# miloknowles/adaptive-stereo-icra-2021

Measured on AMD Instinct MI355X. Metric: stereo pairs/sec (fwd+adapt-step), KITTI 1242x375 D=192, higher is better.
Workload: dtype f32; 1 GPU; KITTI-2015 1242x375, maxdisp 192, k=4 (Dc=12, 24x78 cost volume), forward + one online-adapt step (train-mode BN, monodepth loss, clip 1.0, Adam lr 5e-5); pairs_per_gpu=4, global_batch=4, parallelism=dp1 (per-replica BatchNorm statistics, one flat RCCL gradient all-reduce), kernels=all hand-written HIP (no MIOpen/rocBLAS on the path)

## Files before the change

adaptive-stereo-icra-2021_amd/csrc/conv32_mfma.hip:

```cpp
#include "as_common.h"
#include "conv_epilogue.h"
#include <cstdlib>
#include "conv3d_lds.h"

struct ConvArgs {
  const float* x;
  const float* wp;
  EpilogueArgs ep;
  PclDev gin, gout;
  ConvMap map;
  int M;
  int ntaps;
  int tap_off[AS_MAX_TAPS];
};

__device__ inline void load16(f32x4 (&r)[4], const float* p) {
  const f32x4* q = reinterpret_cast<const f32x4*>(p);
  r[0] = q[0]; r[1] = q[1]; r[2] = q[2]; r[3] = q[3];
}

__device__ inline void loadw(f32x4 (&r)[4], const float* p) {
  r[0] = *reinterpret_cast<const f32x4*>(p);
  r[1] = *reinterpret_cast<const f32x4*>(p + 256);
  r[2] = *reinterpret_cast<const f32x4*>(p + 512);
  r[3] = *reinterpret_cast<const f32x4*>(p + 768);
}

__device__ inline void mfma16(f32x16& acc, const f32x4 (&a)[4], const f32x4 (&b)[4]) {
#pragma unroll
  for (int q = 0; q < 4; ++q) {
    acc = __builtin_amdgcn_mfma_f32_32x32x2f32(a[q].x, b[q].x, acc, 0, 0, 0);
    acc = __builtin_amdgcn_mfma_f32_32x32x2f32(a[q].y, b[q].y, acc, 0, 0, 0);
    acc = __builtin_amdgcn_mfma_f32_32x32x2f32(a[q].z, b[q].z, acc, 0, 0, 0);
    acc = __builtin_amdgcn_mfma_f32_32x32x2f32(a[q].w, b[q].w, acc, 0, 0, 0);
  }
}

#ifndef AS_CONV32_PREFETCH
#define AS_CONV32_PREFETCH 1
#endif
template <int NT>
__device__ __forceinline__ void conv32_fwd_body(const ConvArgs& p, const int block, float (*red)[32], float* bmean) {
  const int lane = threadIdx.x & 63, wave = threadIdx.x >> 6;
  const int h = lane >> 5, li = lane & 31;
  const int tile = block * 4 + wave;
  const int v = tile * 32 + li;
  const bool valid = v < p.M;
  int in_vox, out_vox;
  conv_decode(valid ? v : p.M - 1, p.gin, p.gout, p.map, in_vox, out_vox);

  const float* xa = p.x + (long)in_vox * 32 + h * 16;
  const float* wb = p.wp + lane * 4;

  const float bias_v = p.ep.bias[li];
  __builtin_amdgcn_sched_barrier(0);

  constexpr int PF = AS_CONV32_PREFETCH, RING = PF + 1;
  f32x4 a[RING][4], b[RING][4];
#pragma unroll
  for (int tp = 0; tp < PF && tp < NT; ++tp) {
    load16(a[tp % RING], xa + (long)p.tap_off[tp] * 32);
    loadw(b[tp % RING], wb + tp * 1024);
    __builtin_amdgcn_sched_barrier(0);
  }
  f32x16 acc;
#pragma unroll
  for (int r = 0; r < 16; ++r) acc[r] = bias_v;
#pragma unroll
  for (int tp = 0; tp < NT; ++tp) {
    if (tp + PF < NT) {
      load16(a[(tp + PF) % RING], xa + (long)p.tap_off[tp + PF] * 32);
      loadw(b[(tp + PF) % RING], wb + (tp + PF) * 1024);
    }
    __builtin_amdgcn_sched_barrier(0);
    mfma16(acc, a[tp % RING], b[tp % RING]);
    __builtin_amdgcn_sched_barrier(0);
  }
  TileStats ts;
  conv_epilogue(acc, p.ep, out_vox, valid, min(128, p.M - block * 128), red, bmean, &ts);
  stats_write(p.ep, block, ts);
}

template <int NT>
__global__ __launch_bounds__(256) void conv32_fwd_kernel(ConvArgs p) {
  __shared__ float red[4][32];
  __shared__ float bmean[32];
  conv32_fwd_body<NT>(p, (int)blockIdx.x, red, bmean);
}

struct DgradS2Args { ConvArgs ph[4]; int nblk[4]; };

__global__ __launch_bounds__(256) void conv32_dgrad_s2_kernel(DgradS2Args p) {
  __shared__ float red[4][32];
  __shared__ float bmean[32];
  int b = (int)blockIdx.x;
  if (b < p.nblk[0]) { conv32_fwd_body<9>(p.ph[0], b, red, bmean); return; }
  b -= p.nblk[0];
  if (b < p.nblk[1]) { conv32_fwd_body<6>(p.ph[1], b, red, bmean); return; }
  b -= p.nblk[1];
  if (b < p.nblk[2]) { conv32_fwd_body<6>(p.ph[2], b, red, bmean); return; }
  b -= p.nblk[2];
  conv32_fwd_body<4>(p.ph[3], b, red, bmean);
}

#ifndef CONV32_SPLITK_MAX_M
#define CONV32_SPLITK_MAX_M 32768
#endif
bool conv32_splitk_applies(int ntaps, int64_t M) {
  return (ntaps == 9 && M <= CONV32_SPLITK_MAX_M) || (ntaps == 25 && M <= CONV32_SPLITK_MAX_M / 2);
}

template <int NT>
__global__ __launch_bounds__(256) void conv32_fwd_splitk_kernel(ConvArgs p) {
  __shared__ float red[4][32];
  __shared__ float bmean[32];
  __shared__ float part[3][16][64];
  const int lane = threadIdx.x & 63, wave = __builtin_amdgcn_readfirstlane(threadIdx.x >> 6);
  const int h = lane >> 5, li = lane & 31;
  const int v = blockIdx.x * 32 + li;
  const bool in_range = v < p.M;
  int in_vox, out_vox;
  conv_decode(in_range ? v : p.M - 1, p.gin, p.gout, p.map, in_vox, out_vox);
  const float* xa = p.x + (long)in_vox * 32 + h * 16;
  const float* wb = p.wp + lane * 4;
  const float bias_v = wave == 0 ? p.ep.bias[li] : 0.f;
  constexpr int PER = (NT + 3) / 4;
  f32x4 a[2][4], b[2][4];
  if (wave < NT) {
    load16(a[0], xa + (long)p.tap_off[wave] * 32);
    loadw(b[0], wb + wave * 1024);
  }
  f32x16 acc;
#pragma unroll
  for (int r = 0; r < 16; ++r) acc[r] = bias_v;
#pragma unroll
  for (int k = 0; k < PER; ++k) {
    const int tp = wave + 4 * k;
    if (k + 1 < PER && tp + 4 < NT) {
      load16(a[(k + 1) & 1], xa + (long)p.tap_off[tp + 4] * 32);
      loadw(b[(k + 1) & 1], wb + (tp + 4) * 1024);
    }
    __builtin_amdgcn_sched_barrier(0);
    if (tp < NT) mfma16(acc, a[k & 1], b[k & 1]);
    __builtin_amdgcn_sched_barrier(0);
  }
  if (wave > 0) {
#pragma unroll
    for (int r = 0; r < 16; ++r) part[wave - 1][r][lane] = acc[r];
  }
  __syncthreads();
  if (wave == 0) {
#pragma unroll
    for (int r = 0; r < 16; ++r) acc[r] = ((acc[r] + part[0][r][lane]) + part[1][r][lane]) + part[2][r][lane];
  }
  TileStats ts;
  conv_epilogue(acc, p.ep, out_vox, in_range && wave == 0, min(32, p.M - (int)blockIdx.x * 32), red, bmean, &ts);
  stats_write(p.ep, blockIdx.x, ts);
}

__global__ void pack_weights_kernel(const float* __restrict__ w, float* __restrict__ packed, int T, int flip) {
  const int idx = blockIdx.x * blockDim.x + threadIdx.x;
  if (idx >= T * 1024) return;
  const int e = idx & 3, j = (idx >> 2) & 31, h = (idx >> 7) & 1, q = (idx >> 8) & 3, t = idx >> 10;
  const int k = 16 * h + 4 * q + e;
  float v;
  if (!flip) v = w[((long)j * 32 + k) * T + t];
  else       v = w[((long)k * 32 + j) * T + (T - 1 - t)];
  packed[idx] = v;
}

#define WG_SEG_STEPS 32
template <int TG>
struct WgradAcc { f32x16 a[TG]; };

struct WgradArgs {
  const float* x;
  const float* gz;
  float* partial;
  float* partial_db;
  PclDev gin, gout;
  int rows;
  int nseg;
  int seg_steps;
  int rows_per_chunk;
  int nchunks;
  int ntaps;
  int stride;
  int tap_off[AS_MAX_TAPS];
};

template <int TG>
__global__ __launch_bounds__(256) void conv32_wgrad_kernel(WgradArgs p) {
  extern __shared__ __attribute__((aligned(16))) float lds[];
  const int lane = threadIdx.x & 63, wave = threadIdx.x >> 6;
  const int h = lane >> 5, li = lane & 31;
  int group, chunk;
  {
    const int ngroups = p.ntaps / TG;
    const int L = blockIdx.x, xcd = L & 7, q = L >> 3;
    const int per_xcd = (p.nchunks + 7) >> 3;
    group = q % ngroups;
    chunk = xcd * per_xcd + q / ngroups;
    if (chunk >= p.nchunks || q / ngroups >= per_xcd) return;
  }
  const int W = p.gout.W, H = p.gout.H, D = p.gout.D;
  const int r0 = chunk * p.rows_per_chunk;
  const int r1 = min(p.rows, r0 + p.rows_per_chunk);

  f32x16 acc[TG];
#pragma unroll
  for (int g = 0; g < TG; ++g)
#pragma unroll
    for (int r = 0; r < 16; ++r) acc[g][r] = 0.f;
  float bsum = 0.f;

  int toff[TG];
#pragma unroll
  for (int g = 0; g < TG; ++g) toff[g] = p.tap_off[group * TG + g] * 32;

  constexpr int WG_U = 8;
  const int nsteps = (W + 1) >> 1;
  const int xs = 32 * p.stride;
  for (int unit = r0 + wave; unit < r1; unit += 4) {
    const int row = unit / p.nseg, seg = unit - row * p.nseg;
    int t = row;
    const int y = t % H; t /= H;
    const int d = t % D;
    const int b = t / D;
    const float* xr = p.x + p.gin.vox(b, d, y * p.stride, 0) * 32 + li;
    const float* gr = p.gz + p.gout.vox(b, d, y, 0) * 32 + li;
    const int s_end = min(nsteps, (seg + 1) * p.seg_steps);
    for (int s0 = seg * p.seg_steps; s0 < s_end; s0 += WG_U) {
      float bv[WG_U], av[WG_U][TG];
#pragma unroll
      for (int u = 0; u < WG_U; ++u) {
        const int xc = 2 * (s0 + u) + h;
        const bool ok = xc < W;
        const int xcl = ok ? xc : W - 1;
#ifdef WG_EXP_NOLOAD
        const float g0 = (float)(xcl + lane);
        bv[u] = ok ? g0 : 0.f;
#pragma unroll
        for (int g = 0; g < TG; ++g) av[u][g] = (float)(xcl * xs + toff[g]);
#else
        const float g0 = gr[xcl * 32];
        bv[u] = ok ? g0 : 0.f;
#pragma unroll
        for (int g = 0; g < TG; ++g) av[u][g] = xr[xcl * xs + toff[g]];
#endif
      }
      __builtin_amdgcn_sched_barrier(0);
#pragma unroll
      for (int u = 0; u < WG_U; ++u) {
        bsum += bv[u];
#pragma unroll
        for (int g = 0; g < TG; ++g)
#ifdef WG_EXP_NOMFMA
          acc[g][0] += av[u][g] * bv[u];
#else
          acc[g] = __builtin_amdgcn_mfma_f32_32x32x2f32(av[u][g], bv[u], acc[g], 0, 0, 0);
#endif
      }
    }
  }

  float* slab = lds;
  float* dbs = lds + 3 * TG * 16 * 64;
  bsum += __shfl_xor(bsum, 32, 64);
  if (h == 0) dbs[wave * 32 + li] = bsum;
  if (wave > 0) {
#pragma unroll
    for (int g = 0; g < TG; ++g)
#pragma unroll
      for (int r = 0; r < 16; ++r) slab[((wave - 1) * TG * 16 + g * 16 + r) * 64 + lane] = acc[g][r];
  }
  __syncthreads();
  if (wave == 0) {
#pragma unroll
    for (int g = 0; g < TG; ++g) {
      const int tap = group * TG + g;
      float* out = p.partial + ((long)chunk * p.ntaps + tap) * 1024;
#pragma unroll
      for (int r = 0; r < 16; ++r) {
        float v = acc[g][r];
        v += slab[(0 * TG * 16 + g * 16 + r) * 64 + lane];
        v += slab[(1 * TG * 16 + g * 16 + r) * 64 + lane];
        v += slab[(2 * TG * 16 + g * 16 + r) * 64 + lane];
        const int ci = (r & 3) + 8 * (r >> 2) + 4 * h;
        out[ci * 32 + li] = v;
      }
    }
    if (group == 0 && h == 0)
      p.partial_db[chunk * 32 + li] = dbs[li] + dbs[32 + li] + dbs[64 + li] + dbs[96 + li];
  }
}

__global__ __launch_bounds__(1024) void wgrad_reduce_kernel(const float* __restrict__ partial,
                                                             const float* __restrict__ partial_db, int nchunks, int T,
                                                             float* __restrict__ dW, float* __restrict__ db, int accumulate) {
  __shared__ float red[16][64];
  const int o = threadIdx.x & 63, sl = threadIdx.x >> 6;
  const int total = T * 1024;
  const int idx = blockIdx.x * 64 + o;
  const bool is_w = idx < total, is_b = !is_w && db != nullptr && idx < total + 32;
  float s = 0.f;
  if (is_w) {
    const float* src = partial + idx;
#pragma unroll 8
    for (int c = sl; c < nchunks; c += 16) s += src[(long)c * total];
  } else if (is_b) {
    const float* src = partial_db + (idx - total);
#pragma unroll 8
    for (int c = sl; c < nchunks; c += 16) s += src[c * 32];
  }
  red[sl][o] = s;
  __syncthreads();
  if (sl == 0 && (is_w || is_b)) {
    float t = 0.f;
#pragma unroll
    for (int k = 0; k < 16; ++k) t += red[k][o];
    if (is_w) {
      const int oc = idx & 31, i = (idx >> 5) & 31, tp = idx >> 10;
      float* dst = dW + ((long)oc * 32 + i) * T + tp;
      *dst = accumulate ? *dst + t : t;
    } else {
      db[idx - total] = accumulate ? db[idx - total] + t : t;
    }
  }
}

struct ReduceJob { const float* partial; const float* partial_db; int nchunks, accumulate; };
#define RB_MAX_DEST 32
#define RB_MAX_JOBS 2
struct ReduceDest { float* dW; float* db; int T, njobs; ReduceJob job[RB_MAX_JOBS]; };
struct ReduceBatch { int ndest; ReduceDest dest[RB_MAX_DEST]; };

__global__ __launch_bounds__(1024) void wgrad_reduce_batch_kernel(ReduceBatch rb) {
  __shared__ f32x4 red[16][64];
  const ReduceDest& d = rb.dest[blockIdx.y];
  const int o = threadIdx.x & 63, sl = threadIdx.x >> 6;
  const int total = d.T * 1024;
  const int idx = (blockIdx.x * 64 + o) * 4;
  if (blockIdx.x * 256 >= total + 32) return;
  const bool is_w = idx < total, is_b = !is_w && d.db != nullptr && idx < total + 32;
  f32x4 v = {0.f, 0.f, 0.f, 0.f};
  bool have = false;
  for (int j = 0; j < d.njobs; ++j) {
    const ReduceJob& jb = d.job[j];
    f32x4 s = {0.f, 0.f, 0.f, 0.f};
    if (is_w) {
      const float* src = jb.partial + idx;
#pragma unroll 8
      for (int c = sl; c < jb.nchunks; c += 16) s += *reinterpret_cast<const f32x4*>(src + (long)c * total);
    } else if (is_b) {
      const float* src = jb.partial_db + (idx - total);
#pragma unroll 8
      for (int c = sl; c < jb.nchunks; c += 16) s += *reinterpret_cast<const f32x4*>(src + c * 32);
    }
    __syncthreads();
    red[sl][o] = s;
    __syncthreads();
    if (sl == 0 && (is_w || is_b)) {
      f32x4 t = {0.f, 0.f, 0.f, 0.f};
#pragma unroll
      for (int k = 0; k < 16; ++k) t += red[k][o];
      if (jb.accumulate) {
        if (!have) {
#pragma unroll
          for (int e = 0; e < 4; ++e) {
            const int id = idx + e;
            v[e] = is_w ? d.dW[((long)(id & 31) * 32 + ((id >> 5) & 31)) * d.T + (id >> 10)] : d.db[id - total];
          }
          have = true;
        }
        v = v + t;
      } else { v = t; have = true; }
    }
  }
  if (sl == 0 && (is_w || is_b)) {
#pragma unroll
    for (int e = 0; e < 4; ++e) {
      const int id = idx + e;
      if (is_w) d.dW[((long)(id & 31) * 32 + ((id >> 5) & 31)) * d.T + (id >> 10)] = v[e];
      else d.db[id - total] = v[e];
    }
  }
}

#include <mutex>
#include <vector>
struct PendingReduce { const float* partial; const float* partial_db; int nchunks, T; float* dW; float* db; int accumulate; };
static std::mutex g_defer_mutex;
static bool g_defer_on = false;
static std::vector<PendingReduce> g_defer_jobs;

void as_wgrad_reduce_enqueue(hipStream_t st, const float* partial, const float* partial_db, int nchunks, int T, float* dW,
                             float* db, int accumulate) {
  {
    std::lock_guard<std::mutex> lock(g_defer_mutex);
    if (g_defer_on && accumulate) { g_defer_jobs.push_back({partial, partial_db, nchunks, T, dW, db, accumulate}); return; }
  }
  hipLaunchKernelGGL(wgrad_reduce_kernel, dim3(as_div_up(T * 1024 + 32, 64)), dim3(1024), 0, st, partial, partial_db, nchunks, T,
                     dW, db, accumulate);
}

extern "C" int as_wgrad_defer(int on) {
  std::lock_guard<std::mutex> lock(g_defer_mutex);
  const int prev = g_defer_on ? 1 : 0;
  g_defer_on = on != 0;
  return prev;
}

extern "C" int as_wgrad_defer_pending(void) {
  std::lock_guard<std::mutex> lock(g_defer_mutex);
  return (int)g_defer_jobs.size();
}

static void launch_reduce_batch(const ReduceBatch& rb, hipStream_t st) {
  int tmax = 0;
  for (int i = 0; i < rb.ndest; ++i) tmax = rb.dest[i].T > tmax ? rb.dest[i].T : tmax;
  hipLaunchKernelGGL(wgrad_reduce_batch_kernel, dim3(as_div_up(tmax * 1024 + 32, 256), rb.ndest), dim3(1024), 0, st, rb);
}

extern "C" int as_wgrad_defer_flush(void* stream) {
  std::vector<PendingReduce> jobs;
  {
    std::lock_guard<std::mutex> lock(g_defer_mutex);
    jobs.swap(g_defer_jobs);
  }
  hipStream_t st = (hipStream_t)stream;
  ReduceBatch rb;
  rb.ndest = 0;
  for (const PendingReduce& pj : jobs) {
    int di = -1;
    for (int i = 0; i < rb.ndest; ++i) if (rb.dest[i].dW == pj.dW) di = i;
    if (di >= 0 && (rb.dest[di].njobs == RB_MAX_JOBS || rb.dest[di].T != pj.T || rb.dest[di].db != pj.db)) {
      launch_reduce_batch(rb, st);
      rb.ndest = 0; di = -1;
    }
    if (di < 0) {
      if (rb.ndest == RB_MAX_DEST) { launch_reduce_batch(rb, st); rb.ndest = 0; }
      di = rb.ndest++;
      rb.dest[di].dW = pj.dW; rb.dest[di].db = pj.db; rb.dest[di].T = pj.T; rb.dest[di].njobs = 0;
    }
    ReduceJob& jb = rb.dest[di].job[rb.dest[di].njobs++];
    jb.partial = pj.partial; jb.partial_db = pj.partial_db; jb.nchunks = pj.nchunks; jb.accumulate = pj.accumulate;
  }
// ... 103 lines not shown
    for (int px = 0; px < 2; ++px, ++ph) {
      const int Hl = (ggx->H - py + 1) / 2, Wl = (ggx->W - px + 1) / 2;
      ConvArgs& a = args.ph[ph];
      int n = 0;
      for (int j = py; j < 5; j += 2)
        for (int l = px; l < 5; l += 2) {
          a.tap_off[n] = ((py + 2 - j) / 2) * Wp + (px + 2 - l) / 2;
          ++n;
        }
      a.x = f.x; a.wp = wp; a.ep = epilogue_args(f);
      a.gin = as_make_dev(ggz); a.gout = as_make_dev(ggx);
      a.map.Hl = Hl > 0 ? Hl : 1; a.map.Wl = Wl > 0 ? Wl : 1; a.map.in_stride = 1; a.map.out_stride = 2; a.map.out_oy = py; a.map.out_ox = px;
      a.M = (Hl > 0 && Wl > 0) ? ggx->B * Hl * Wl : 0; a.ntaps = n;
      args.nblk[ph] = as_div_up(a.M, 128);
      total += args.nblk[ph];
      wp += n * 1024;
    }
  if (total > 0) hipLaunchKernelGGL(conv32_dgrad_s2_kernel, dim3(total), dim3(256), 0, (hipStream_t)stream, args);
  return AS_OK;
}

extern "C" int as_conv32_pack_weights(const float* w, float* packed, const as_conv_shape* s,
                                      int transpose_flip, void* stream) {
  AS_CHECK_ARG(w && packed && s, "as_conv32_pack_weights: null pointer");
  const int T = s->kd * s->kh * s->kw;
  AS_CHECK_ARG(T >= 1 && T <= AS_MAX_TAPS, "as_conv32_pack_weights: %d taps unsupported", T);
  hipLaunchKernelGGL(pack_weights_kernel, dim3(as_div_up(T * 1024, 256)), dim3(256), 0, (hipStream_t)stream,
                     w, packed, T, transpose_flip);
  AS_CHECK_LAUNCH("as_conv32_pack_weights");
  return AS_OK;
}

__device__ inline int s2_phase_major_tap(int t) {
  int n = 0;
  for (int py = 0; py < 2; ++py)
    for (int px = 0; px < 2; ++px)
      for (int j = py; j < 5; j += 2)
        for (int l = px; l < 5; l += 2) { if (n == t) return j * 5 + l; ++n; }
  return 0;
}

__device__ inline float wino_g_row(int r, float x0, float x1, float x2) {
  return r == 0 ? x0 : (r == 3 ? x2 : (r == 1 ? 0.5f * ((x0 + x2) + x1) : 0.5f * ((x0 + x2) - x1)));
}
__device__ inline void wino_pack_one(const float* __restrict__ w, float* __restrict__ packed, int idx, bool transposed) {
  if (idx >= 16 * 1024) return;
  const int e = idx & 3, j = (idx >> 2) & 31, h = (idx >> 7) & 1, q = (idx >> 8) & 3, kk = idx >> 10;
  const int k = 16 * h + 4 * q + e, r = kk >> 2, c = kk & 3;
  const float* g = transposed ? w + ((long)k * 32 + j) * 9 : w + ((long)j * 32 + k) * 9;
  float col[3];
#pragma unroll
  for (int a = 0; a < 3; ++a) {
    const float* ga = g + 3 * (transposed ? 2 - a : a);
    col[a] = transposed ? wino_g_row(c, ga[2], ga[1], ga[0]) : wino_g_row(c, ga[0], ga[1], ga[2]);
  }
  packed[idx] = wino_g_row(r, col[0], col[1], col[2]);
}
__global__ void wino_pack_kernel(const float* __restrict__ w, float* __restrict__ packed, int transposed) {
  wino_pack_one(w, packed, blockIdx.x * blockDim.x + threadIdx.x, transposed != 0);
}

__global__ void pack_weights_batch_kernel(const as_pack_job* __restrict__ jobs) {
  const as_pack_job job = jobs[blockIdx.y];
  const int T = job.taps, kind = job.transpose_flip;
  const int idx = blockIdx.x * blockDim.x + threadIdx.x;
  if (kind >= AS_PACK_CONV4 && kind < AS_PACK_CONV4 + 8) {
    const int Cin = kind - AS_PACK_CONV4;
    if (idx >= T * 128) return;
    const int co = idx & 31, h = (idx >> 5) & 1, j = (idx >> 6) & 1, t = idx >> 7;
    const int c = 2 * j + h;
    job.packed[idx] = c < Cin ? job.w[((long)co * Cin + c) * T + t] : 0.f;
    return;
  }
  if (kind == AS_PACK_MIRROR_TAP || kind == AS_PACK_MIRROR_CH) {
    if (idx >= 288) return;
    const int c = idx / 9, t = idx - 9 * c;
    const float v = job.w[((long)c * 4) * 9 + (8 - t)];
    job.packed[kind == AS_PACK_MIRROR_TAP ? t * 32 + c : c * 9 + t] = v;
    return;
  }
  if (kind == AS_PACK_WINO || kind == AS_PACK_WINO_T) { wino_pack_one(job.w, job.packed, idx, kind == AS_PACK_WINO_T); return; }
  if (idx >= T * 1024) return;
  const int e = idx & 3, j = (idx >> 2) & 31, h = (idx >> 7) & 1, q = (idx >> 8) & 3, t = idx >> 10;
  const int k = 16 * h + 4 * q + e;
  if (kind == AS_PACK_S2_DGRAD) job.packed[idx] = job.w[((long)k * 32 + j) * T + s2_phase_major_tap(t)];
  else job.packed[idx] = kind ? job.w[((long)k * 32 + j) * T + (T - 1 - t)] : job.w[((long)j * 32 + k) * T + t];
}

extern "C" int as_conv32_pack_weights_batch(const as_pack_job* jobs, int njobs, int max_taps, void* stream) {
  AS_CHECK_ARG(jobs && njobs >= 1 && njobs <= 65535, "as_conv32_pack_weights_batch: bad job table");
  AS_CHECK_ARG(max_taps >= 1 && max_taps <= AS_MAX_TAPS, "as_conv32_pack_weights_batch: %d taps unsupported", max_taps);
  hipLaunchKernelGGL(pack_weights_batch_kernel, dim3(as_div_up(max_taps * 1024, 256), njobs), dim3(256), 0,
                     (hipStream_t)stream, jobs);
  AS_CHECK_LAUNCH("as_conv32_pack_weights_batch");
  return AS_OK;
}

extern "C" int as_conv32_wino_pack_weights(const float* w, float* packed, int transposed, void* stream) {
  AS_CHECK_ARG(w && packed, "as_conv32_wino_pack_weights: null pointer");
  hipLaunchKernelGGL(wino_pack_kernel, dim3(64), dim3(256), 0, (hipStream_t)stream, w, packed, transposed);
  AS_CHECK_LAUNCH("as_conv32_wino_pack_weights");
  return AS_OK;
}

extern "C" int as_conv3d_wgrad_lds_assignment(int ntiles, int nchunks, int block, int* chunk, int* kd, int* extra_tile) {
  AS_CHECK_ARG(chunk && kd && extra_tile && ntiles >= 1 && nchunks >= 1 && nchunks <= ntiles && block >= 0,
               "as_conv3d_wgrad_lds_assignment: bad arguments");
  return conv3d_wgrad_assign(block, ntiles, nchunks, chunk, kd, extra_tile) ? 1 : 0;
}

Wgrad32Plan conv32_wgrad_plan(const as_pcl* gout, const as_conv_shape* s) {
  Wgrad32Plan p;
  p.T = s->kd * s->kh * s->kw;
  p.tap_group = (p.T % 3 == 0) ? 3 : (p.T % 5 == 0 ? 5 : 1);
  const int groups = p.T / p.tap_group;
  const int nsteps = (gout->W + 1) >> 1;
  const long waves = (long)gout->B * gout->D * gout->H * groups;
  int nseg = 1;
  if (waves < 1024) {
    nseg = (int)((2048 + waves - 1) / waves);
    const int most = (nsteps + WG_SEG_STEPS - 1) / WG_SEG_STEPS;
    if (nseg > most) nseg = most;
    if (nseg < 1) nseg = 1;
  }
  int steps = (nsteps + nseg - 1) / nseg;
  p.seg_steps = (steps + 7) / 8 * 8;
  p.nseg = (nsteps + p.seg_steps - 1) / p.seg_steps;
  const int rows = gout->B * gout->D * gout->H * p.nseg;
  int want_chunks = (4096 + groups * 4 - 1) / (groups * 4);
  if (want_chunks > 512) want_chunks = 512;
  p.rows_per_chunk = (rows + want_chunks - 1) / want_chunks;
  if (p.rows_per_chunk < 4) p.rows_per_chunk = 4;
  p.nchunks = (rows + p.rows_per_chunk - 1) / p.rows_per_chunk;
  return p;
}

template <int TG>
static void launch_wgrad(const WgradArgs& a, int groups, int nchunks, hipStream_t st) {
  const size_t lds = (size_t)(3 * TG * 16 * 64 + 4 * 32) * sizeof(float);
  const int per_xcd = (nchunks + 7) / 8;
  hipLaunchKernelGGL(conv32_wgrad_kernel<TG>, dim3(8 * per_xcd * groups), dim3(256), lds, st, a);
}

int conv32_wgrad_generic_launch(const ConvWgradArgs& w, const as_pcl* gin, const as_pcl* gout, const as_conv_shape* s,
                                const Wgrad32Plan& p, const char* who, void* stream) {
  WgradArgs a;
  a.x = w.x; a.gz = w.gz; a.partial = w.partial; a.partial_db = w.partial_db;
  a.gin = as_make_dev(gin); a.gout = as_make_dev(gout);
  a.nseg = p.nseg; a.seg_steps = p.seg_steps;
  a.rows = gout->B * gout->D * gout->H * a.nseg; a.rows_per_chunk = p.rows_per_chunk; a.nchunks = p.nchunks; a.ntaps = p.T;
  a.stride = s->stride;
  if (int e = fill_taps(gin, s, a.tap_off, who)) return e;
  hipStream_t st = (hipStream_t)stream;
  if (p.tap_group == 3) launch_wgrad<3>(a, p.T / 3, p.nchunks, st);
  else if (p.tap_group == 5) launch_wgrad<5>(a, p.T / 5, p.nchunks, st);
  else launch_wgrad<1>(a, p.T, p.nchunks, st);
  return AS_OK;
}
```

adaptive-stereo-icra-2021_amd/csrc/conv32_s2.hip:

```cpp
#include "as_common.h"
#include "conv_entry.h"

struct S2Args {
  const float* x;
  const float* wp;
  const float* bias;
  float* out;
  PclDev gin, gout;
  int nseg, ntiles;
};

__device__ inline void s2_loadw(f32x4 (&r)[4], const float* p) {
  r[0] = *reinterpret_cast<const f32x4*>(p);
  r[1] = *reinterpret_cast<const f32x4*>(p + 256);
  r[2] = *reinterpret_cast<const f32x4*>(p + 512);
  r[3] = *reinterpret_cast<const f32x4*>(p + 768);
}
__device__ inline void s2_mfma16(f32x16& acc, const f32x4 (&a)[4], const f32x4 (&b)[4]) {
#pragma unroll
  for (int q = 0; q < 4; ++q) {
    acc = __builtin_amdgcn_mfma_f32_32x32x2f32(a[q].x, b[q].x, acc, 0, 0, 0);
    acc = __builtin_amdgcn_mfma_f32_32x32x2f32(a[q].y, b[q].y, acc, 0, 0, 0);
    acc = __builtin_amdgcn_mfma_f32_32x32x2f32(a[q].z, b[q].z, acc, 0, 0, 0);
    acc = __builtin_amdgcn_mfma_f32_32x32x2f32(a[q].w, b[q].w, acc, 0, 0, 0);
  }
}

#define S2F_HALF (36 * 128)
#define S2F_BUF (2 * S2F_HALF)
#define S2F_WAVE (2 * S2F_BUF)

__global__ __launch_bounds__(256, 2) void conv32_s2_fwd_kernel(S2Args p) {
  extern __shared__ __attribute__((aligned(16))) char smem_s2[];
  const int lane = threadIdx.x & 63, wave = threadIdx.x >> 6;
  const int h = lane >> 5, li = lane & 31;
  const int tile = blockIdx.x * 4 + wave;
  if (tile >= p.ntiles) return;
  const int seg = tile % p.nseg, row = tile / p.nseg;
  const int y = row % p.gout.H, b = row / p.gout.H;
  const int x0 = seg * 32;
  char* buf = smem_s2 + wave * S2F_WAVE;

  const int sv = lane >> 3, sq = lane & 7;
  const int s_half = (sv & 1) * S2F_HALF;
  const float* src0 = p.x + ((((long)b * p.gin.Hp + (2 * y - 2 + p.gin.ph)) * p.gin.Wp + (2 * x0 - 2 + p.gin.pw)) * 32) + sq * 4;
  const int vlim = p.gin.Wp - 1 - (2 * x0 - 2 + p.gin.pw);
  int voff[9];
#pragma unroll
  for (int i = 0; i < 9; ++i) voff[i] = min(8 * i + sv, vlim) * 32;
  auto fetch = [&](f32x4 (&r)[9], int ky) {
    const float* src = src0 + (long)ky * p.gin.Wp * 32;
#pragma unroll
    for (int i = 0; i < 9; ++i) r[i] = *reinterpret_cast<const f32x4*>(src + voff[i]);
  };
  auto stage = [&](const f32x4 (&r)[9], char* dst) {
#pragma unroll
    for (int i = 0; i < 9; ++i) {
      const int e = 4 * i + (sv >> 1);
      *reinterpret_cast<f32x4*>(dst + s_half + e * 128 + ((sq ^ ((e >> 1) & 7)) << 4)) = r[i];
    }
  };
  const float* wb = p.wp + lane * 4;
  const float bias_v = p.bias ? p.bias[li] : 0.f;
  f32x16 acc;
#pragma unroll
  for (int r = 0; r < 16; ++r) acc[r] = bias_v;

  f32x4 ra[9], rb[9];
  f32x4 bw[2][4];
  fetch(ra, 0);
  s2_loadw(bw[0], wb);
#pragma unroll
  for (int ky = 0; ky < 5; ++ky) {
    char* cur = buf + (ky & 1) * S2F_BUF;
    if (ky & 1) stage(rb, cur); else stage(ra, cur);
    if (ky + 1 < 5) { if (ky & 1) fetch(ra, ky + 1); else fetch(rb, ky + 1); }
#pragma unroll
    for (int kx = 0; kx < 5; ++kx) {
      const int tp = ky * 5 + kx;
      if (tp + 1 < 25) s2_loadw(bw[(tp + 1) & 1], wb + (tp + 1) * 1024);
      f32x4 a[4];
      const int e = li + (kx >> 1);
      const char* ap = cur + (kx & 1) * S2F_HALF + e * 128;
      const int sw = (e >> 1) & 7;
#pragma unroll
      for (int q = 0; q < 4; ++q) a[q] = *reinterpret_cast<const f32x4*>(ap + (((4 * h + q) ^ sw) << 4));
      __builtin_amdgcn_sched_barrier(0);
      s2_mfma16(acc, a, bw[tp & 1]);
      __builtin_amdgcn_sched_barrier(0);
    }
  }
  float* outp = p.out + ((((long)b * p.gout.Hp + (y + p.gout.ph)) * p.gout.Wp + (x0 + p.gout.pw)) * 32) + li;
#pragma unroll
  for (int r = 0; r < 16; ++r) {
    const int xo = (r & 3) + 8 * (r >> 2) + 4 * h;
    if (x0 + xo < p.gout.W) outp[xo * 32] = acc[r];
  }
}

bool conv32_s2_fwd_applicable(const as_pcl* gin, const as_pcl* gout, const as_conv_shape* s) {
  if (s->kd != 1 || s->kh != 5 || s->kw != 5 || s->stride != 2 || s->dil != 1 || s->pad_h != 2 || s->pad_w != 2) return false;
  if (gin->D != 1 || gout->D != 1 || gin->pd != 0 || gin->B != gout->B) return false;
  if (gout->H != (gin->H - 1) / 2 + 1 || gout->W != (gin->W - 1) / 2 + 1) return false;
  if (gin->ph < 2 || gin->pw < 2) return false;
  return (long)gout->B * gout->H * ((gout->W + 31) / 32) >= 1024;
}

int conv32_s2_fwd_launch(const ConvFwdArgs& f, const as_pcl* gin, const as_pcl* gout, const as_conv_shape*, const char* who,
                         void* stream) {
  static AsPerDevice attr_set;
  S2Args a;
  a.x = f.x; a.wp = f.w; a.bias = f.bias; a.out = f.z; a.gin = as_make_dev(gin); a.gout = as_make_dev(gout);
  a.nseg = (gout->W + 31) / 32; a.ntiles = gout->B * gout->H * a.nseg;
  void* kargs[] = {&a};
  return as_launch_lds(reinterpret_cast<const void*>(conv32_s2_fwd_kernel), attr_set, 4 * S2F_WAVE, 4 * S2F_WAVE,
                       dim3(as_div_up(a.ntiles, 4)), dim3(256), kargs, who, (hipStream_t)stream);
}

#define S2D_ROW (40 * 128)
#define S2D_WAVE (3 * S2D_ROW)

__global__ __launch_bounds__(256, 2) void conv32_s2_dgrad_kernel(S2Args p) {
  extern __shared__ __attribute__((aligned(16))) char smem_s2[];
  const int lane = threadIdx.x & 63, wave = threadIdx.x >> 6;
  const int h = lane >> 5, li = lane & 31;
  const int tile = blockIdx.x * 4 + wave;
  if (tile >= p.ntiles) return;
  const int seg = tile % p.nseg, row = tile / p.nseg;
  const int yc = row % p.gin.H, b = row / p.gin.H;
  const int x0 = seg * 32;
  char* buf = smem_s2 + wave * S2D_WAVE;

  const int sv = lane >> 3, sq = lane & 7;
  const float* src0 = p.x + ((((long)b * p.gin.Hp + (yc - 1 + p.gin.ph)) * p.gin.Wp + (x0 - 1 + p.gin.pw)) * 32) + sq * 4;
  const int vlim = p.gin.Wp - 1 - (x0 - 1 + p.gin.pw);
  int voff[5];
#pragma unroll
  for (int i = 0; i < 5; ++i) voff[i] = min(8 * i + sv, vlim) * 32;
  f32x4 r[3][5];
#pragma unroll
  for (int dy = 0; dy < 3; ++dy)
#pragma unroll
    for (int i = 0; i < 5; ++i) r[dy][i] = *reinterpret_cast<const f32x4*>(src0 + (long)dy * p.gin.Wp * 32 + voff[i]);
  const float* wb = p.wp + lane * 4;
  f32x4 bw[2][4];
  s2_loadw(bw[0], wb);
#pragma unroll
  for (int dy = 0; dy < 3; ++dy)
#pragma unroll
    for (int i = 0; i < 5; ++i) {
      const int e = 8 * i + sv;
      *reinterpret_cast<f32x4*>(buf + dy * S2D_ROW + e * 128 + ((sq ^ ((e >> 1) & 7)) << 4)) = r[dy][i];
    }

  int tp = 0;
#pragma unroll
  for (int ph = 0; ph < 4; ++ph) {
    const int py = ph >> 1, px = ph & 1;
    f32x16 acc;
#pragma unroll
    for (int rr = 0; rr < 16; ++rr) acc[rr] = 0.f;
#pragma unroll
    for (int j = py; j < 5; j += 2)
#pragma unroll
      for (int l = px; l < 5; l += 2, ++tp) {
        if (tp + 1 < 25) s2_loadw(bw[(tp + 1) & 1], wb + (tp + 1) * 1024);
        const int dy = (py + 2 - j) / 2 + 1, dx = (px + 2 - l) / 2;
        const int e = li + 1 + dx;
        const char* ap = buf + dy * S2D_ROW + e * 128;
        const int sw = (e >> 1) & 7;
        f32x4 a[4];
#pragma unroll
        for (int q = 0; q < 4; ++q) a[q] = *reinterpret_cast<const f32x4*>(ap + (((4 * h + q) ^ sw) << 4));
        __builtin_amdgcn_sched_barrier(0);
        s2_mfma16(acc, a, bw[tp & 1]);
        __builtin_amdgcn_sched_barrier(0);
      }
    const int yo = 2 * yc + py;
    if (yo < p.gout.H) {
      float* outp = p.out + ((((long)b * p.gout.Hp + (yo + p.gout.ph)) * p.gout.Wp + (2 * x0 + px + p.gout.pw)) * 32) + li;
#pragma unroll
      for (int rr = 0; rr < 16; ++rr) {
        const int xo = (rr & 3) + 8 * (rr >> 2) + 4 * h;
        if (2 * (x0 + xo) + px < p.gout.W) outp[xo * 64] = acc[rr];
      }
    }
  }
}

bool conv32_s2_dgrad_applicable(const as_pcl* ggz, const as_pcl* ggx) {
  if (ggz->D != 1 || ggx->D != 1 || ggz->B != ggx->B || ggz->pd != 0) return false;
  if (ggz->H != (ggx->H - 1) / 2 + 1 || ggz->W != (ggx->W - 1) / 2 + 1) return false;
  if (ggz->ph < 1 || ggz->pw < 1) return false;
  return (long)ggz->B * ggz->H * ((ggz->W + 31) / 32) >= 1024;
}

int conv32_s2_dgrad_launch(const float* gz, const as_pcl* ggz, const float* packed, float* gx, const as_pcl* ggx, const char* who,
                           void* stream) {
  static AsPerDevice attr_set;
  S2Args a;
  a.x = gz; a.wp = packed; a.bias = nullptr; a.out = gx; a.gin = as_make_dev(ggz); a.gout = as_make_dev(ggx);
  a.nseg = (ggz->W + 31) / 32; a.ntiles = ggz->B * ggz->H * a.nseg;
  void* kargs[] = {&a};
  return as_launch_lds(reinterpret_cast<const void*>(conv32_s2_dgrad_kernel), attr_set, 4 * S2D_WAVE, 4 * S2D_WAVE,
                       dim3(as_div_up(a.ntiles, 4)), dim3(256), kargs, who, (hipStream_t)stream);
}
```

Baseline: 588.2 stereo pairs/s.

## Process two tiles per wave in stride-2 conv kernels with persistent grid

The stride-2 forward and dgrad kernels now use a persistent grid capped at 512 blocks, with each wave taking a contiguous range of work units. Each unit computes two output tiles and shares the weight loads between them: forward handles two adjacent tiles, dgrad handles two input rows that reuse overlapping staged rows. This cuts weight-fetch traffic and launch overhead per tile. In exchange each wave holds more registers and two accumulators, which may lower occupancy, and fixed static work splitting can leave waves unevenly loaded. Optional per-wave cycle-timing instrumentation is also added, compiled out by default.

```diff
diff --git a/adaptive-stereo-icra-2021_amd/csrc/conv32_mfma.hip b/adaptive-stereo-icra-2021_amd/csrc/conv32_mfma.hip
--- a/adaptive-stereo-icra-2021_amd/csrc/conv32_mfma.hip
+++ b/adaptive-stereo-icra-2021_amd/csrc/conv32_mfma.hip
@@ -2,6 +2,7 @@
 #include "conv_epilogue.h"
 #include <cstdlib>
 #include "conv3d_lds.h"
+#include "s2_timing.h"
 
 struct ConvArgs {
   const float* x;
@@ -187,6 +188,9 @@
   int ntaps;
   int stride;
   int tap_off[AS_MAX_TAPS];
+#ifdef S2_TIMING_BUILD
+  long long* timing;
+#endif
 };
 
 template <int TG>
@@ -221,6 +225,7 @@
   constexpr int WG_U = 8;
   const int nsteps = (W + 1) >> 1;
   const int xs = 32 * p.stride;
+  S2_T_BEGIN;
   for (int unit = r0 + wave; unit < r1; unit += 4) {
     const int row = unit / p.nseg, seg = unit - row * p.nseg;
     int t = row;
@@ -250,6 +255,9 @@
 #endif
       }
       __builtin_amdgcn_sched_barrier(0);
+      S2_T(0);
+      S2_WAIT_VM(0);
+      S2_T(1);
 #pragma unroll
       for (int u = 0; u < WG_U; ++u) {
         bsum += bv[u];
@@ -261,6 +269,7 @@
           acc[g] = __builtin_amdgcn_mfma_f32_32x32x2f32(av[u][g], bv[u], acc[g], 0, 0, 0);
 #endif
       }
+      S2_T(2);
     }
   }
 
@@ -293,6 +302,9 @@
     if (group == 0 && h == 0)
       p.partial_db[chunk * 32 + li] = dbs[li] + dbs[32 + li] + dbs[64 + li] + dbs[96 + li];
   }
+  S2_WAIT_VM(0);
+  S2_T(3);
+  S2_T_END(p.timing, blockIdx.x * 4 + wave, (r1 - r0 - wave + 3) / 4);
 }
 
 __global__ __launch_bounds__(1024) void wgrad_reduce_kernel(const float* __restrict__ partial,
@@ -702,8 +714,15 @@
   a.stride = s->stride;
   if (int e = fill_taps(gin, s, a.tap_off, who)) return e;
   hipStream_t st = (hipStream_t)stream;
+#ifdef S2_TIMING_BUILD
+  static long long* timing_buf = nullptr;
+  a.timing = as_timing_begin(timing_buf, S2_TIMING_BYTES, st);
+#endif
   if (p.tap_group == 3) launch_wgrad<3>(a, p.T / 3, p.nchunks, st);
   else if (p.tap_group == 5) launch_wgrad<5>(a, p.T / 5, p.nchunks, st);
   else launch_wgrad<1>(a, p.T, p.nchunks, st);
-  return AS_OK;
-}
+#ifdef S2_TIMING_BUILD
+  if (p.tap_group == 5) s2_timing_dump("wgrad", timing_buf, st);
+#endif
+  return AS_OK;
+}
diff --git a/adaptive-stereo-icra-2021_amd/csrc/conv32_s2.hip b/adaptive-stereo-icra-2021_amd/csrc/conv32_s2.hip
--- a/adaptive-stereo-icra-2021_amd/csrc/conv32_s2.hip
+++ b/adaptive-stereo-icra-2021_amd/csrc/conv32_s2.hip
@@ -1,5 +1,8 @@
 #include "as_common.h"
 #include "conv_entry.h"
+#include "s2_timing.h"
+
+#define S2_GRID 512
 
 struct S2Args {
   const float* x;
@@ -8,13 +11,18 @@
   float* out;
   PclDev gin, gout;
   int nseg, ntiles;
+  int nunits;
+#ifdef S2_TIMING_BUILD
+  long long* timing;
+#endif
 };
 
-__device__ inline void s2_loadw(f32x4 (&r)[4], const float* p) {
-  r[0] = *reinterpret_cast<const f32x4*>(p);
-  r[1] = *reinterpret_cast<const f32x4*>(p + 256);
-  r[2] = *reinterpret_cast<const f32x4*>(p + 512);
-  r[3] = *reinterpret_cast<const f32x4*>(p + 768);
+__device__ inline f32x4 s2_ld(const float* base, unsigned lane_bytes, int imm_bytes = 0) {
+  return *reinterpret_cast<const f32x4*>(reinterpret_cast<const char*>(base) + lane_bytes + imm_bytes);
+}
+__device__ inline void s2_loadw(f32x4 (&r)[4], const float* tap, unsigned lane_bytes) {
+#pragma unroll
+  for (int q = 0; q < 4; ++q) r[q] = s2_ld(tap, lane_bytes, q * 1024);
 }
 __device__ inline void s2_mfma16(f32x16& acc, const f32x4 (&a)[4], const f32x4 (&b)[4]) {
 #pragma unroll
@@ -25,6 +33,12 @@
     acc = __builtin_amdgcn_mfma_f32_32x32x2f32(a[q].w, b[q].w, acc, 0, 0, 0);
   }
 }
+__device__ inline void s2_share(int nunits, int& first, int& end, int& gw) {
+  gw = __builtin_amdgcn_readfirstlane(blockIdx.x * 4 + (threadIdx.x >> 6));
+  const int nw = gridDim.x * 4;
+  first = (int)((long)nunits * gw / nw);
+  end = (int)((long)nunits * (gw + 1) / nw);
+}
 
 #define S2F_HALF (36 * 128)
 #define S2F_BUF (2 * S2F_HALF)
@@ -34,68 +48,106 @@
   extern __shared__ __attribute__((aligned(16))) char smem_s2[];
   const int lane = threadIdx.x & 63, wave = threadIdx.x >> 6;
   const int h = lane >> 5, li = lane & 31;
-  const int tile = blockIdx.x * 4 + wave;
-  if (tile >= p.ntiles) return;
-  const int seg = tile % p.nseg, row = tile / p.nseg;
-  const int y = row % p.gout.H, b = row / p.gout.H;
-  const int x0 = seg * 32;
   char* buf = smem_s2 + wave * S2F_WAVE;
-
   const int sv = lane >> 3, sq = lane & 7;
-  const int s_half = (sv & 1) * S2F_HALF;
-  const float* src0 = p.x + ((((long)b * p.gin.Hp + (2 * y - 2 + p.gin.ph)) * p.gin.Wp + (2 * x0 - 2 + p.gin.pw)) * 32) + sq * 4;
-  const int vlim = p.gin.Wp - 1 - (2 * x0 - 2 + p.gin.pw);
-  int voff[9];
-#pragma unroll
-  for (int i = 0; i < 9; ++i) voff[i] = min(8 * i + sv, vlim) * 32;
-  auto fetch = [&](f32x4 (&r)[9], int ky) {
-    const float* src = src0 + (long)ky * p.gin.Wp * 32;
-#pragma unroll
-    for (int i = 0; i < 9; ++i) r[i] = *reinterpret_cast<const f32x4*>(src + voff[i]);
-  };
-  auto stage = [&](const f32x4 (&r)[9], char* dst) {
-#pragma unroll
-    for (int i = 0; i < 9; ++i) {
-      const int e = 4 * i + (sv >> 1);
-      *reinterpret_cast<f32x4*>(dst + s_half + e * 128 + ((sq ^ ((e >> 1) & 7)) << 4)) = r[i];
+  int s_off[4];
+#pragma unroll
+  for (int j = 0; j < 4; ++j) s_off[j] = (sv & 1) * S2F_HALF + (sv >> 1) * 128 + ((sq ^ ((2 * j + (sv >> 2)) & 7)) << 4);
+  const unsigned wl = lane * 16;
+  const float bias_v = p.bias ? p.bias[li] : 0.f;
+  int u, u_end, gw;
+  s2_share(p.nunits, u, u_end, gw);
+  (void)gw;
+  S2_T_BEGIN;
+#ifdef S2_TIMING_BUILD
+  const int u_first = u;
+#endif
+
+  for (; u < u_end; ++u) {
+    int wz = 0;
+    asm volatile("" : "+s"(wz));
+    const float* wp = p.wp + wz;
+    const float* src0[2];
+    float* outp[2];
+    int vlimb[2];
+    int xlim[2];
+#pragma unroll
+    for (int t = 0; t < 2; ++t) {
+      const int tile = min(2 * u + t, p.ntiles - 1);
+      const int seg = tile % p.nseg, row = tile / p.nseg;
+      const int y = row % p.gout.H, b = row / p.gout.H;
+      const int x0 = seg * 32;
+      src0[t] = p.x + ((((long)b * p.gin.Hp + (2 * y - 2 + p.gin.ph)) * p.gin.Wp + (2 * x0 - 2 + p.gin.pw)) * 32);
+      vlimb[t] = (p.gin.Wp - 1 - (2 * x0 - 2 + p.gin.pw)) * 128;
+      outp[t] = p.out + ((((long)b * p.gout.Hp + (y + p.gout.ph)) * p.gout.Wp + (x0 + p.gout.pw)) * 32);
+      xlim[t] = 2 * u + t < p.ntiles ? p.gout.W - x0 : 0;
     }
-  };
-  const float* wb = p.wp + lane * 4;
-  const float bias_v = p.bias ? p.bias[li] : 0.f;
-  f32x16 acc;
-#pragma unroll
-  for (int r = 0; r < 16; ++r) acc[r] = bias_v;
-
-  f32x4 ra[9], rb[9];
-  f32x4 bw[2][4];
-  fetch(ra, 0);
-  s2_loadw(bw[0], wb);
-#pragma unroll
-  for (int ky = 0; ky < 5; ++ky) {
-    char* cur = buf + (ky & 1) * S2F_BUF;
-    if (ky & 1) stage(rb, cur); else stage(ra, cur);
-    if (ky + 1 < 5) { if (ky & 1) fetch(ra, ky + 1); else fetch(rb, ky + 1); }
-#pragma unroll
-    for (int kx = 0; kx < 5; ++kx) {
-      const int tp = ky * 5 + kx;
-      if (tp + 1 < 25) s2_loadw(bw[(tp + 1) & 1], wb + (tp + 1) * 1024);
-      f32x4 a[4];
-      const int e = li + (kx >> 1);
-      const char* ap = cur + (kx & 1) * S2F_HALF + e * 128;
-      const int sw = (e >> 1) & 7;
-#pragma unroll
-      for (int q = 0; q < 4; ++q) a[q] = *reinterpret_cast<const f32x4*>(ap + (((4 * h + q) ^ sw) << 4));
-      __builtin_amdgcn_sched_barrier(0);
-      s2_mfma16(acc, a, bw[tp & 1]);
-      __builtin_amdgcn_sched_barrier(0);
+    auto fetch = [&](f32x4 (&r)[9], int t, int ky) {
+      const float* src = src0[t] + (long)ky * p.gin.Wp * 32;
+      int svb = sv * 128;
+      asm volatile("" : "+v"(svb));
+#pragma unroll
+      for (int i = 0; i < 9; ++i) r[i] = s2_ld(src, (unsigned)(min(svb + i * 1024, vlimb[t]) + sq * 16));
+    };
+    auto stage = [&](const f32x4 (&r)[9], char* dst) {
+#pragma unroll
+      for (int i = 0; i < 9; ++i) *reinterpret_cast<f32x4*>(dst + s_off[i & 3] + i * 512) = r[i];
+    };
+    f32x16 acc[2];
+#pragma unroll
+    for (int t = 0; t < 2; ++t)
+#pragma unroll
+      for (int r = 0; r < 16; ++r) acc[t][r] = bias_v;
+
+    f32x4 rr[2][9];
+    f32x4 bw[2][4];
+    fetch(rr[0], 0, 0);
+    fetch(rr[1], 1, 0);
+    s2_loadw(bw[0], wp, wl);
+#pragma unroll
+    for (int ky = 0; ky < 5; ++ky) {
+      S2_T(1);
+      S2_WAIT_VM(4);
+      S2_T(0);
+      stage(rr[0], buf);
+      stage(rr[1], buf + S2F_BUF);
+      if (ky + 1 < 5) { fetch(rr[0], 0, ky + 1); fetch(rr[1], 1, ky + 1); }
+#pragma unroll
+      for (int kx = 0; kx < 5; ++kx) {
+        const int tp = ky * 5 + kx;
+        if (tp + 1 < 25) s2_loadw(bw[(tp + 1) & 1], wp + (tp + 1) * 1024, wl);
+        f32x4 a[2][4];
+        const int e = li + (kx >> 1);
+        const int sw = (e >> 1) & 7;
+#pragma unroll
+        for (int t = 0; t < 2; ++t) {
+          const char* ap = buf + t * S2F_BUF + (kx & 1) * S2F_HALF + e * 128;
+#pragma unroll
+          for (int q = 0; q < 4; ++q) a[t][q] = *reinterpret_cast<const f32x4*>(ap + (((4 * h + q) ^ sw) << 4));
+        }
+        S2_T(1);
+        S2_WAIT_LGKM();
+        S2_T(2);
+        if (tp == 24) S2_WAIT_VM(0); else if (kx == 0 && ky < 4) S2_WAIT_VM(22); else S2_WAIT_VM(4);
+        S2_T(3);
+        __builtin_amdgcn_sched_barrier(0);
+        s2_mfma16(acc[0], a[0], bw[tp & 1]);
+        s2_mfma16(acc[1], a[1], bw[tp & 1]);
+        __builtin_amdgcn_sched_barrier(0);
+        S2_T(4);
+      }
     }
+#pragma unroll
+    for (int t = 0; t < 2; ++t)
+#pragma unroll
+      for (int r = 0; r < 16; ++r) {
+        const int xo = (r & 3) + 8 * (r >> 2) + 4 * h;
+        if (xo < xlim[t]) outp[t][xo * 32 + li] = acc[t][r];
+      }
+    S2_WAIT_VM(0);
+    S2_T(5);
   }
-  float* outp = p.out + ((((long)b * p.gout.Hp + (y + p.gout.ph)) * p.gout.Wp + (x0 + p.gout.pw)) * 32) + li;
-#pragma unroll
-  for (int r = 0; r < 16; ++r) {
-    const int xo = (r & 3) + 8 * (r >> 2) + 4 * h;
-    if (x0 + xo < p.gout.W) outp[xo * 32] = acc[r];
-  }
+  S2_T_END(p.timing, gw, 2 * (u_end - u_first));
 }
 
 bool conv32_s2_fwd_applicable(const as_pcl* gin, const as_pcl* gout, const as_conv_shape* s) {
@@ -106,86 +158,133 @@
   return (long)gout->B * gout->H * ((gout->W + 31) / 32) >= 1024;
 }
 
+static dim3 s2_grid(int nunits) { const int g = as_div_up(nunits, 4); return dim3(g < S2_GRID ? g : S2_GRID); }
+
 int conv32_s2_fwd_launch(const ConvFwdArgs& f, const as_pcl* gin, const as_pcl* gout, const as_conv_shape*, const char* who,
                          void* stream) {
   static AsPerDevice attr_set;
   S2Args a;
   a.x = f.x; a.wp = f.w; a.bias = f.bias; a.out = f.z; a.gin = as_make_dev(gin); a.gout = as_make_dev(gout);
   a.nseg = (gout->W + 31) / 32; a.ntiles = gout->B * gout->H * a.nseg;
+  a.nunits = (a.ntiles + 1) / 2;
+#ifdef S2_TIMING_BUILD
+  static long long* timing_buf = nullptr;
+  a.timing = as_timing_begin(timing_buf, S2_TIMING_BYTES, (hipStream_t)stream);
+#endif
   void* kargs[] = {&a};
-  return as_launch_lds(reinterpret_cast<const void*>(conv32_s2_fwd_kernel), attr_set, 4 * S2F_WAVE, 4 * S2F_WAVE,
-                       dim3(as_div_up(a.ntiles, 4)), dim3(256), kargs, who, (hipStream_t)stream);
-}
-
-#define S2D_ROW (40 * 128)
-#define S2D_WAVE (3 * S2D_ROW)
+  const int e = as_launch_lds(reinterpret_cast<const void*>(conv32_s2_fwd_kernel), attr_set, 4 * S2F_WAVE, 4 * S2F_WAVE,
+                              s2_grid(a.nunits), dim3(256), kargs, who, (hipStream_t)stream);
+#ifdef S2_TIMING_BUILD
+  if (!e) s2_timing_dump("fwd", timing_buf, (hipStream_t)stream);
+#endif
+  return e;
+}
+
+#define S2D_ROW (36 * 128)
+#define S2D_WAVE (4 * S2D_ROW)
 
 __global__ __launch_bounds__(256, 2) void conv32_s2_dgrad_kernel(S2Args p) {
   extern __shared__ __attribute__((aligned(16))) char smem_s2[];
   const int lane = threadIdx.x & 63, wave = threadIdx.x >> 6;
   const int h = lane >> 5, li = lane & 31;
-  const int tile = blockIdx.x * 4 + wave;
-  if (tile >= p.ntiles) return;
-  const int seg = tile % p.nseg, row = tile / p.nseg;
-  const int yc = row % p.gin.H, b = row / p.gin.H;
-  const int x0 = seg * 32;
   char* buf = smem_s2 + wave * S2D_WAVE;
-
   const int sv = lane >> 3, sq = lane & 7;
-  const float* src0 = p.x + ((((long)b * p.gin.Hp + (yc - 1 + p.gin.ph)) * p.gin.Wp + (x0 - 1 + p.gin.pw)) * 32) + sq * 4;
-  const int vlim = p.gin.Wp - 1 - (x0 - 1 + p.gin.pw);
-  int voff[5];
-#pragma unroll
-  for (int i = 0; i < 5; ++i) voff[i] = min(8 * i + sv, vlim) * 32;
-  f32x4 r[3][5];
-#pragma unroll
-  for (int dy = 0; dy < 3; ++dy)
-#pragma unroll
-    for (int i = 0; i < 5; ++i) r[dy][i] = *reinterpret_cast<const f32x4*>(src0 + (long)dy * p.gin.Wp * 32 + voff[i]);
-  const float* wb = p.wp + lane * 4;
-  f32x4 bw[2][4];
-  s2_loadw(bw[0], wb);
-#pragma unroll
-  for (int dy = 0; dy < 3; ++dy)
-#pragma unroll
-    for (int i = 0; i < 5; ++i) {
-      const int e = 8 * i + sv;
-      *reinterpret_cast<f32x4*>(buf + dy * S2D_ROW + e * 128 + ((sq ^ ((e >> 1) & 7)) << 4)) = r[dy][i];
+  const unsigned wl = lane * 16;
+  const int H = p.gin.H, rp = (H + 1) >> 1;
+  int u, u_end, gw;
+  s2_share(p.nunits, u, u_end, gw);
+  (void)gw;
+  S2_T_BEGIN;
+#ifdef S2_TIMING_BUILD
+  const int u_first = u;
+#endif
+
+  for (; u < u_end; ++u) {
+    const int seg = u % p.nseg, row = u / p.nseg;
+    const int yc = 2 * (row % rp), b = row / rp;
+    const int x0 = seg * 32;
+    int wz = 0;
+    asm volatile("" : "+s"(wz));
+    const float* wp = p.wp + wz;
+    const float* src0 = p.x + ((((long)b * p.gin.Hp + (yc - 1 + p.gin.ph)) * p.gin.Wp + (x0 - 1 + p.gin.pw)) * 32);
+    const int vlim = p.gin.Wp - 1 - (x0 - 1 + p.gin.pw);
+    unsigned voff[5];
+#pragma unroll
+    for (int i = 0; i < 5; ++i) voff[i] = (unsigned)(min(8 * i + sv, vlim) * 128 + sq * 16);
+    const int dy3 = min(yc + 2, H) - (yc - 1);
+    f32x4 r[4][5];
+#pragma unroll
+    for (int dy = 0; dy < 4; ++dy)
+#pragma unroll
+      for (int i = 0; i < 5; ++i)
+        if (i < 4 || sv < 4) r[dy][i] = s2_ld(src0 + (long)(dy < 3 ? dy : dy3) * p.gin.Wp * 32, voff[i]);
+    f32x4 bw[2][4];
+    s2_loadw(bw[0], wp, wl);
+    S2_T(1);
+    S2_WAIT_VM(4);
+    S2_T(0);
+#pragma unroll
+    for (int dy = 0; dy < 4; ++dy)
+#pragma unroll
+      for (int i = 0; i < 5; ++i) {
+        const int e = 8 * i + sv;
+        if (i < 4 || sv < 4) *reinterpret_cast<f32x4*>(buf + dy * S2D_ROW + e * 128 + ((sq ^ ((e >> 1) & 7)) << 4)) = r[dy][i];
+      }
+
+    int tp = 0;
+#pragma unroll
+    for (int ph = 0; ph < 4; ++ph) {
+      const int py = ph >> 1, px = ph & 1;
+      f32x16 acc[2];
+#pragma unroll
+      for (int t = 0; t < 2; ++t)
+#pragma unroll
+        for (int q = 0; q < 16; ++q) acc[t][q] = 0.f;
+#pragma unroll
+      for (int j = py; j < 5; j += 2)
+#pragma unroll
+        for (int l = px; l < 5; l += 2, ++tp) {
+          if (tp + 1 < 25) s2_loadw(bw[(tp + 1) & 1], wp + (tp + 1) * 1024, wl);
+          const int dy = (py + 2 - j) / 2 + 1, dx = (px + 2 - l) / 2;
+          const int e = li + 1 + dx;
+          const int sw = (e >> 1) & 7;
+          f32x4 a[2][4];
+#pragma unroll
+          for (int t = 0; t < 2; ++t) {
+            const char* ap = buf + (dy + t) * S2D_ROW + e * 128;
+#pragma unroll
+            for (int q = 0; q < 4; ++q) a[t][q] = *reinterpret_cast<const f32x4*>(ap + (((4 * h + q) ^ sw) << 4));
+          }
+          S2_T(1);
+          S2_WAIT_LGKM();
+          S2_T(2);
+          S2_WAIT_VM(4);
+          S2_T(3);
+          __builtin_amdgcn_sched_barrier(0);
+          s2_mfma16(acc[0], a[0], bw[tp & 1]);
+          s2_mfma16(acc[1], a[1], bw[tp & 1]);
+          __builtin_amdgcn_sched_barrier(0);
+          S2_T(4);
+        }
+#pragma unroll
+      for (int t = 0; t < 2; ++t) {
+        const int yo = 2 * (yc + t) + py;
+        if (yo < p.gout.H) {
+          float* outp = p.out + ((((long)b * p.gout.Hp + (yo + p.gout.ph)) * p.gout.Wp + (2 * x0 + px + p.gout.pw)) * 32);
+#pragma unroll
+          for (int q = 0; q < 16; ++q) {
+            const int xo = (q & 3) + 8 * (q >> 2) + 4 * h;
+            if (2 * (x0 + xo) + px < p.gout.W) outp[xo * 64 + li] = acc[t][q];
+          }
+        }
+      }
+      S2_WAIT_VM(4);
+      S2_T(5);
     }
-
-  int tp = 0;
-#pragma unroll
-  for (int ph = 0; ph < 4; ++ph) {
-    const int py = ph >> 1, px = ph & 1;
-    f32x16 acc;
-#pragma unroll
-    for (int rr = 0; rr < 16; ++rr) acc[rr] = 0.f;
-#pragma unroll
-    for (int j = py; j < 5; j += 2)
-#pragma unroll
-      for (int l = px; l < 5; l += 2, ++tp) {
-        if (tp + 1 < 25) s2_loadw(bw[(tp + 1) & 1], wb + (tp + 1) * 1024);
-        const int dy = (py + 2 - j) / 2 + 1, dx = (px + 2 - l) / 2;
-        const int e = li + 1 + dx;
-        const char* ap = buf + dy * S2D_ROW + e * 128;
-        const int sw = (e >> 1) & 7;
-        f32x4 a[4];
-#pragma unroll
-        for (int q = 0; q < 4; ++q) a[q] = *reinterpret_cast<const f32x4*>(ap + (((4 * h + q) ^ sw) << 4));
-        __builtin_amdgcn_sched_barrier(0);
-        s2_mfma16(acc, a, bw[tp & 1]);
-        __builtin_amdgcn_sched_barrier(0);
-      }
-    const int yo = 2 * yc + py;
-    if (yo < p.gout.H) {
-      float* outp = p.out + ((((long)b * p.gout.Hp + (yo + p.gout.ph)) * p.gout.Wp + (2 * x0 + px + p.gout.pw)) * 32) + li;
-#pragma unroll
-      for (int rr = 0; rr < 16; ++rr) {
-        const int xo = (rr & 3) + 8 * (rr >> 2) + 4 * h;
-        if (2 * (x0 + xo) + px < p.gout.W) outp[xo * 64] = acc[rr];
-      }
-    }
+    S2_WAIT_VM(0);
+    S2_T(5);
   }
+  S2_T_END(p.timing, gw, 2 * (u_end - u_first));
 }
 
 bool conv32_s2_dgrad_applicable(const as_pcl* ggz, const as_pcl* ggx) {
@@ -201,7 +300,16 @@
   S2Args a;
   a.x = gz; a.wp = packed; a.bias = nullptr; a.out = gx; a.gin = as_make_dev(ggz); a.gout = as_make_dev(ggx);
   a.nseg = (ggz->W + 31) / 32; a.ntiles = ggz->B * ggz->H * a.nseg;
+  a.nunits = ggz->B * ((ggz->H + 1) / 2) * a.nseg;
+#ifdef S2_TIMING_BUILD
+  static long long* timing_buf = nullptr;
+  a.timing = as_timing_begin(timing_buf, S2_TIMING_BYTES, (hipStream_t)stream);
+#endif
   void* kargs[] = {&a};
-  return as_launch_lds(reinterpret_cast<const void*>(conv32_s2_dgrad_kernel), attr_set, 4 * S2D_WAVE, 4 * S2D_WAVE,
-                       dim3(as_div_up(a.ntiles, 4)), dim3(256), kargs, who, (hipStream_t)stream);
-}
+  const int e = as_launch_lds(reinterpret_cast<const void*>(conv32_s2_dgrad_kernel), attr_set, 4 * S2D_WAVE, 4 * S2D_WAVE,
+                              s2_grid(a.nunits), dim3(256), kargs, who, (hipStream_t)stream);
+#ifdef S2_TIMING_BUILD
+  if (!e) s2_timing_dump("dgrad", timing_buf, (hipStream_t)stream);
+#endif
+  return e;
+}
diff --git a/adaptive-stereo-icra-2021_amd/csrc/s2_timing.h b/adaptive-stereo-icra-2021_amd/csrc/s2_timing.h
--- /dev/null
+++ b/adaptive-stereo-icra-2021_amd/csrc/s2_timing.h
@@ -0,0 +1,30 @@
+#pragma once
+#ifdef S2_TIMING_BUILD
+#include <cstdio>
+#include "conv32_layer.h"
+
+#define S2_TIMING_WAVES 16384
+#define S2_TIMING_BYTES ((size_t)S2_TIMING_WAVES * 8 * sizeof(long long))
+#define S2_T_BEGIN long long tacc[8] = {0, 0, 0, 0, 0, 0, 0, 0}; long long tlast = clock64(); const long long wall0 = wall_clock64()
+#define S2_T(slot) do { __builtin_amdgcn_sched_barrier(0); const long long now_ = clock64(); tacc[slot] += now_ - tlast; \
+                        tlast = now_; __builtin_amdgcn_sched_barrier(0); } while (0)
+#define S2_WAIT_VM(n) asm volatile("s_waitcnt vmcnt(" #n ")" ::: "memory")
+#define S2_WAIT_LGKM() asm volatile("s_waitcnt lgkmcnt(0)" ::: "memory")
+#define S2_T_END(buf, gwave, units) do { if ((buf) && (threadIdx.x & 63) == 0 && (gwave) < S2_TIMING_WAVES) { \
+    long long* o_ = (buf) + (long)(gwave) * 8; for (int i_ = 0; i_ < 6; ++i_) o_[i_] = tacc[i_]; \
+    o_[6] = wall_clock64() - wall0; o_[7] = (units); } } while (0)
+
+static inline void s2_timing_dump(const char* kernel, const long long* buf, hipStream_t st) {
+  const char* dir = getenv("AS_S2_TIMING");
+  void* hbuf = as_timing_fetch("AS_S2_TIMING", buf, S2_TIMING_BYTES, st);
+  if (!hbuf) return;
+  char name[512]; snprintf(name, sizeof name, "%s/s2_timing_%s.bin", dir, kernel);
+  FILE* f = fopen(name, "wb"); if (f) { fwrite(hbuf, 1, S2_TIMING_BYTES, f); fclose(f); } free(hbuf);
+}
+#else
+#define S2_T_BEGIN do { } while (0)
+#define S2_T(slot) do { } while (0)
+#define S2_WAIT_VM(n) do { } while (0)
+#define S2_WAIT_LGKM() do { } while (0)
+#define S2_T_END(buf, gwave, units) do { } while (0)
+#endif
```

After: 586.0 stereo pairs/s. About the same (-0.4%).
